# CSU-KangHu/HiTE

Measured on AMD Instinct MI355X. Metric: candidate TE boundaries/sec on 1 Gbp synthetic genome (fine stage: copy finding+gather+align+vote+judge), higher is better.
Workload: dtype u8; 1 GPU; C3: 1000 Mbp synthetic genome, 2500 TIR + 2500 LTR families, 50000 candidates/GPU judged as TIR (copy finding by minimizer-index lookup inside the timed step; index build 0.0 s untimed); genome_bp=1000000000, candidates_per_gpu=50000, candidate_bases=192511237, copies=799813, copy_table=found, is_te=34225, parallelism=replicated genome, candidates per rank x1, all-gather of 32-B calls

## Files before the change

hite_amd/_lib.py:

```python
import ctypes as C
import os

import numpy as np

_HERE = os.path.dirname(os.path.abspath(__file__))
SO_PATH = os.path.join(_HERE, "libhite_gpu.so")

HITE_TE = {"tir": 0, "helitron": 1, "non_ltr": 2}
INFO = {0: "", 1: "nb", 2: "fl1", 3: "EXC"}
HITE_SUBCLUSTER_CHUNK = 64
LTRDEEP_PARAMS, LTRDEEP_ROWS, LTRDEEP_COLS, LTRDEEP_KMER = 40026, 100, 200, 3872


class HiteError(RuntimeError):
    pass


class HiteCall(C.Structure):
    _fields_ = [("is_te", C.c_int32), ("info", C.c_int32), ("row_num", C.c_int32), ("bstart", C.c_int32),
                ("bend", C.c_int32), ("cons_len", C.c_int32), ("cons_off", C.c_int64)]


CALL_DTYPE = np.dtype([("is_te", "<i4"), ("info", "<i4"), ("row_num", "<i4"), ("bstart", "<i4"), ("bend", "<i4"),
                       ("cons_len", "<i4"), ("cons_off", "<i8")])
# ... 42 lines not shown

    def __init__(self, device=0):
        self.lib = load()
        h = C.c_void_p()
        rc = self.lib.hite_ctx_create(int(device), C.byref(h))
        if rc != 0:
            raise HiteError("hite_ctx_create(device=%d) failed: %d (no usable GPU?)" % (device, rc))
        self.h = h
        self.device = device

    def copy_config(self, aligned_interval):
        self._check(self.lib.hite_copy_config_ctx(self.h, -1 if aligned_interval is None else int(bool(aligned_interval))), "hite_copy_config_ctx")

    def fill_config(self, tiles):
        self._check(self.lib.hite_fill_config_ctx(self.h, -1 if tiles is None else int(bool(tiles))), "hite_fill_config_ctx")

    def fill_tile_limits(self):
        out = (C.c_int32 * 4)()
        self._check(self.lib.hite_fill_tile_limits(out), "hite_fill_tile_limits")
        return tuple(out)

    def release_copy_index(self):
        if getattr(self, "_copy_state", None) is not None and getattr(self, "h", None):
            self.lib.hite_copy_index_release(self._copy_state)
        self._copy_state = None

    def close(self):
        self.release_copy_index()
        for lib in list(getattr(self, "_prot_libs", ())) + list(getattr(self, "_ltr_models", ())):
            lib.release()
# ... 1057 lines not shown
```

hite_amd/csrc/hite_align.h:

```cpp
#pragma once
#include "hite_common.h"

int hite_align_run(hite_ctx *ctx, int32_t n_cand, const uint8_t *d_win, const int64_t *d_win_off, const int32_t *d_win_len,
                   const int32_t *d_row_first, int64_t total_rows, const int64_t *d_ops_base, uint16_t *d_ops,
                   int32_t *d_row_dead, int32_t *d_cand_flag, int32_t *d_info, const char *tag, hipStream_t st);
void hite_align_release(hite_ctx *ctx);
```

hite_amd/csrc/hite_align.hip:

```cpp
#include "hite_common.h"
#include "hite_scan.h"
#include "hite_arena.h"
#include "hite_sort.h"
#include "hite_align.h"

#define AL_GAP 3
#define AL_STEER 24
#define AL_MARGIN 48
#define AL_PADR 1056
#define AL_WIDE_NW 64
#define AL_STRIP 16
#define AL_RECB 4096
#define AL_DEFAULT_CAP 8
#define AL_KBINS 2048
#define AL_LANES_MIN_STRIPS 32

struct AlignArgs {
    const uint8_t *win;
    const int64_t *win_off;
    const int32_t *win_len;
    const int32_t *row_first;
    int n_cand;
    const int32_t *row_cand;
    const uint4 *planes;
// ... 1239 lines not shown
                    i -= ups;
                    if (i > 0) {
                        if ((dgv >> ps) & 1ull) { out.put(i - 1, (uint32_t)(j - 1)); i--; j--; }
                        else j--;
                    }
                }
            }
        }
        __syncthreads();
    }
    if (fail) { if (lane == 0) P.st[g] = 1; }
    else out.run(i - 1, i, 0x8000u);
}

__global__ void align_flag_kernel(int64_t nrows, const int32_t *__restrict__ order, const int32_t *__restrict__ strips, AlignArgs P,
                                  int what, int level, int cap, int32_t *__restrict__ flag, int32_t *__restrict__ cols) {
    const int64_t x = (int64_t)blockIdx.x * blockDim.x + threadIdx.x;
    if (x >= nrows) return;
    const int g = order[x];
    int f = 0;
    if (strips[g] > 0) {
        if (what == 0) {
            const int u4 = P.U4[g];
            if (P.st[g] == 0 && u4 >= 0 && u4 + AL_GAP * AL_MARGIN <= 32 * AL_GAP * cap) {
                int first = 8;
                while (32 * AL_GAP * first < u4 + AL_GAP * AL_MARGIN) first *= 2;
                const bool cert = P.U[g] <= P.kst[g];
                f = level >= first && !cert;
            }
        } else if (what == 1) f = P.st[g] == 1;
        else {
            const int u4 = P.U4[g];
            const bool esc = P.st[g] == 0 && u4 >= 0 && u4 + AL_GAP * AL_MARGIN <= 32 * AL_GAP * cap && !(P.U[g] <= P.kst[g]);
            f = what == 2 ? esc : !esc;
        }
    }
    flag[x] = f;
    if (cols) cols[x] = f ? P.win_len[g] + 1 : 0;
}
__global__ void align_compact_kernel(int64_t nrows, const int32_t *__restrict__ order, const int32_t *__restrict__ flag,
                                     const int64_t *__restrict__ pos, int32_t *__restrict__ out, const int64_t *__restrict__ colpos,
                                     int64_t *__restrict__ full_off, int32_t *__restrict__ st) {
    const int64_t x = (int64_t)blockIdx.x * blockDim.x + threadIdx.x;
    if (x >= nrows) return;
    if (flag[x]) {
        const int g = order[x];
        out[pos[x]] = g;
        if (full_off) { full_off[g] = colpos[x]; st[g] = 0; }
    }
}
__global__ void __launch_bounds__(256) align_blockmax_kernel(int64_t cnt, const int32_t *__restrict__ list, const int32_t *__restrict__ strips,
                                                             int32_t *__restrict__ bk) {
    const int64_t x = (int64_t)blockIdx.x * 256 + threadIdx.x;
    const int k = wave_max_i32(x < cnt ? strips[list[x]] : 0);
    if ((threadIdx.x & 63) == 0 && x < cnt) bk[x >> 6] = k;
}
__global__ void align_assign_kernel(int64_t cnt, const int32_t *__restrict__ list, const int64_t *__restrict__ boff, char *region,
                                    unsigned long long *__restrict__ rec) {
    const int64_t x = (int64_t)blockIdx.x * blockDim.x + threadIdx.x;
    if (x < cnt) rec[list[x]] = (unsigned long long)(uintptr_t)(region + boff[x >> 6] * (int64_t)AL_RECB + (x & 63) * 32);
}
struct LaneCost { float thread_chain, lane_chain, thread_work, lane_work; };
__device__ __forceinline__ double lane_cost_at(int64_t k, int64_t nb, const int32_t *bk, const int64_t *boff, const LaneCost c) {
    const double chain_l = k > 0 ? (double)bk[0] * c.lane_chain : 0.0, chain_t = k < nb ? (double)bk[k] * c.thread_chain : 0.0;
// ... 70 lines not shown
    info[g * 5 + 3] = P.kst[g];
    info[g * 5 + 4] = P.lvl[g];
}

struct AlignState {
    Arena arena;
    int64_t *h_pin = nullptr;
    int64_t *d_scal = nullptr;
    int exact_cap = -1;
    int lanes_min = -1;
    float lanes_scale[4] = {1.f, 1.f, 1.f, 1.f};
    bool sort_attr = false;
    hipStream_t st2 = nullptr;
    hipEvent_t ev = nullptr, ev_fork = nullptr, ev_join = nullptr;
    int64_t stats[8] = {0, 0, 0, 0, 0, 0, 0, 0};
};

static hipError_t align_make_stream(hipStream_t *out) {
    int lo = 0, hi = 0;
    if (hipDeviceGetStreamPriorityRange(&lo, &hi) != hipSuccess) { lo = 0; hi = 0; }
    return hipStreamCreateWithPriority(out, hipStreamNonBlocking, hi);
}

static AlignState *align_state(hite_ctx *ctx) {
    if (!ctx->align_state) {
        AlignState *S = new AlignState();
        if (hipHostMalloc((void **)&S->h_pin, 64 * sizeof(int64_t)) != hipSuccess || hipMalloc((void **)&S->d_scal, 64 * sizeof(int64_t)) != hipSuccess ||
            align_make_stream(&S->st2) != hipSuccess || hipEventCreateWithFlags(&S->ev, hipEventDisableTiming) != hipSuccess ||
            hipEventCreateWithFlags(&S->ev_fork, hipEventDisableTiming) != hipSuccess || hipEventCreateWithFlags(&S->ev_join, hipEventDisableTiming) != hipSuccess) {
            delete S;
// ... 49 lines not shown
    return HITE_OK;
}

#define ACHK(x) do { int rc__ = (x); if (rc__) return rc__; } while (0)

template <typename T>
static int aalloc(hite_ctx *ctx, Arena &A, size_t count, T **out) {
    void *p = nullptr;
    int rc = arena_alloc(ctx, A, count * sizeof(T), &p);
    *out = (T *)p;
    return rc;
}

static int build_list(hite_ctx *ctx, AlignState *S, hipStream_t st, int64_t nrows, const int32_t *order, const int32_t *strips,
                      AlignArgs &P, int what, int level, int cap, int32_t *flag, int32_t *cols, int64_t *pos, int64_t *colpos,
                      int64_t *scan_tmp, int32_t *list, int64_t *full_off, int64_t *count, int64_t *total_cols, int slot = 0) {
    const unsigned nb = (unsigned)((nrows + 255) / 256);
    hipLaunchKernelGGL(align_flag_kernel, dim3(nb), dim3(256), 0, st, nrows, order, strips, P, what, level, cap, flag, cols);
    ACHK(scan_excl_buf<int32_t>(ctx, scan_tmp, flag, nrows, pos, st));
    if (cols) ACHK(scan_excl_buf<int32_t>(ctx, scan_tmp, cols, nrows, colpos, st));
    hipLaunchKernelGGL(align_compact_kernel, dim3(nb), dim3(256), 0, st, nrows, order, flag, pos, list, cols ? colpos : nullptr,
                       cols ? full_off : nullptr, P.st);
    HITE_CHECK(ctx, hipMemcpyAsync(S->d_scal + slot, pos + nrows, 8, hipMemcpyDeviceToDevice, st));
    if (cols) HITE_CHECK(ctx, hipMemcpyAsync(S->d_scal + slot + 1, colpos + nrows, 8, hipMemcpyDeviceToDevice, st));
    HITE_CHECK(ctx, hipMemcpyAsync(S->h_pin + slot, S->d_scal + slot, 16, hipMemcpyDeviceToHost, st));
    HITE_CHECK(ctx, hipStreamSynchronize(st));
    *count = S->h_pin[slot];
    if (total_cols) *total_cols = cols ? S->h_pin[slot + 1] : 0;
    return HITE_OK;
}

static int assign_records(hite_ctx *ctx, AlignState *S, hipStream_t st, const int32_t *list, int64_t cnt, const int32_t *strips, int32_t *bk,
                          int64_t *boff, int64_t *scan_tmp, unsigned long long *rec, int slot, int words = 4, int64_t *n_long = nullptr, int64_t *n_long_tb = nullptr) {
    if (n_long) *n_long = 0;
    if (n_long_tb) *n_long_tb = 0;
    if (cnt <= 0) return HITE_OK;
    const int64_t nb = (cnt + 63) / 64;
    hipLaunchKernelGGL(align_blockmax_kernel, dim3((unsigned)((cnt + 255) / 256)), dim3(256), 0, st, cnt, list, strips, bk);
    ACHK(scan_excl_buf<int32_t>(ctx, scan_tmp, bk, nb, boff, st));
    HITE_CHECK(ctx, hipMemcpyAsync(S->d_scal + slot, boff + nb, 8, hipMemcpyDeviceToDevice, st));
    const bool lanes = n_long && S->lanes_min != -2;
    if (lanes) {
        LaneCost fwd4 = {5440.f, 3200.f, 4.3f, 12.5f}, fwd8 = {7040.f, 3200.f, 13.75f, 25.f}, tb = {6880.f, 530.f, 4.3f, 21.5f};
// ... 4 lines not shown
    }
    HITE_CHECK(ctx, hipMemcpyAsync(S->h_pin + slot, S->d_scal + slot, 24, hipMemcpyDeviceToHost, st));
    HITE_CHECK(ctx, hipStreamSynchronize(st));
    const int64_t block_strips = S->h_pin[slot];
    if (lanes) {
        const int64_t v = S->h_pin[slot + 1] * 64, vt = S->h_pin[slot + 2] * 64;
        *n_long = v < cnt ? v : cnt;
        if (n_long_tb) *n_long_tb = vt < cnt ? vt : cnt;
    }
    char *region;
    ACHK(aalloc(ctx, S->arena, (size_t)block_strips * AL_RECB + 256, &region));
    hipLaunchKernelGGL(align_assign_kernel, dim3((unsigned)((cnt + 255) / 256)), dim3(256), 0, st, cnt, list, boff, region, rec);
    return HITE_OK;
}

int hite_align_run(hite_ctx *ctx, int32_t n_cand, const uint8_t *d_win, const int64_t *d_win_off, const int32_t *d_win_len,
                   const int32_t *d_row_first, int64_t total_rows, const int64_t *d_ops_base, uint16_t *d_ops,
                   int32_t *d_row_dead, int32_t *d_cand_flag, int32_t *d_info, const char *tag, hipStream_t st) {
    if (!ctx || n_cand < 0 || total_rows < 0 || total_rows > 0x7fffffff) return HITE_EINVAL;
    if (n_cand == 0 || total_rows == 0) return HITE_OK;
    AlignState *S = align_state(ctx);
    if (!S) return HITE_ENOMEM;
    Arena &A = S->arena;
    ACHK(arena_reset(ctx, A, true));
    const int cap = S->exact_cap;
    AlignArgs P;
    memset(&P, 0, sizeof P);
    P.win = d_win; P.win_off = d_win_off; P.win_len = d_win_len; P.row_first = d_row_first; P.n_cand = n_cand;
    P.ops_base = d_ops_base; P.ops = d_ops;
    int32_t *row_cand, *strips, *order, *pwords, *flag, *flag2, *cols, *list, *list_esc, *list_fin;
    unsigned long long *skeys;
    int64_t *plane_off, *pos, *pos2, *colpos, *scan_tmp, *scan_tmp2, *full_off, *boff, *boff2;
    int32_t *bk, *bk2;
    unsigned long long *rec;
// ... 140 lines not shown
            snprintf(lname, sizeof lname, "align_tb_strips%s", tag ? tag : "");
            const int tl = hite_prof_begin(ctx, lname, s2);
            hipLaunchKernelGGL(align_tb_strips_kernel, dim3((unsigned)nltb), dim3(64), 0, s2, P, order, (int)nltb);
            hite_prof_end(ctx, tl, s2);
            HITE_CHECK(ctx, hipEventRecord(S->ev_join, s2));
        }
        if (nrows > nltb) {
            tk = hite_prof_begin(ctx, name, st);
            hipLaunchKernelGGL(align_tb_kernel, dim3((unsigned)((nrows - nltb + 63) / 64)), dim3(64), 0, st, P, order + nltb, (int)(nrows - nltb));
            hite_prof_end(ctx, tk, st);
        }
        if (nltb > 0) HITE_CHECK(ctx, hipStreamWaitEvent(st, S->ev_join, 0));
    }
    HITE_CHECK(ctx, hipGetLastError());
    {
        int64_t cnt = 0, tcols = 0;
        ACHK(build_list(ctx, S, st, total_rows, order, strips, P, 1, 0, cap, flag, cols, pos, colpos, scan_tmp, list, full_off, &cnt, &tcols));
        if (cnt > 0) {
            tk = hite_prof_begin(ctx, "align_fallback", st);
            ACHK(aalloc(ctx, A, (size_t)tcols * 2 * AL_WIDE_NW + 64, &P.fullbuf));
            ACHK(aalloc(ctx, A, (size_t)tcols + 16, &P.fullt));
            hipLaunchKernelGGL(align_wide_fwd_kernel, dim3((unsigned)cnt), dim3(64), 0, st, P, list, (int)cnt);
            hipLaunchKernelGGL(align_wide_tb_kernel, dim3((unsigned)cnt), dim3(64), 0, st, P, list, (int)cnt);
            hite_prof_end(ctx, tk, st);
        }
    }
    HITE_CHECK(ctx, hipMemsetAsync(S->d_scal, 0, 64, st));
    hipLaunchKernelGGL(align_stats_kernel, dim3((unsigned)(total_rows + 255 < 1024 * 256 ? (total_rows + 255) / 256 : 1024)), dim3(256), 0, st, total_rows, strips, P, d_row_dead, d_cand_flag,
                       (unsigned long long *)S->d_scal);
    if (d_info) hipLaunchKernelGGL(align_info_kernel, dim3((unsigned)((total_rows + 255) / 256)), dim3(256), 0, st, total_rows, P, d_info);
    HITE_CHECK(ctx, hipMemcpyAsync(S->h_pin, S->d_scal, 56, hipMemcpyDeviceToHost, st));
    HITE_CHECK(ctx, hipStreamSynchronize(st));
    for (int q = 0; q < 7; q++) S->stats[q] += S->h_pin[q];
    HITE_CHECK(ctx, hipGetLastError());
    return HITE_OK;
}
```

hite_amd/csrc/hite_common.h:

```cpp
#pragma once
#include <hip/hip_runtime.h>
#include <stdint.h>
#include <stdio.h>
#include <string.h>
#include <stdlib.h>
#include "../../include/hite_gpu.h"

#define HITE_WAVE 64
#define HITE_BLOCK 256

#define JUDGE_CLS_BLOCK 0
#define JUDGE_CLS_WAVE 1
#define JUDGE_CLS_LDS 2
#define JUDGE_LDS_WAVE_SIZES 3
#define JUDGE_LDS_BLOCK_SIZES 2
#define JUDGE_NCLS (JUDGE_CLS_LDS + JUDGE_LDS_WAVE_SIZES + JUDGE_LDS_BLOCK_SIZES)
#define HITE_AUX_STREAMS (JUDGE_NCLS - 1)
struct JudgeFuse {
    const uint8_t *win;
    const int64_t *win_off;
    const int32_t *win_len;
    const int32_t *row_first;
    const int64_t *ops_base;
    const uint16_t *ops;
// ... 22 lines not shown
    int prof_on;
    int prof_n;
    char prof_name[64][32];
    double prof_ms[64];
    int64_t prof_count[64];
    int prof_pending;
    void *prof_ev[512][2];
    int prof_stage[512];
    void *align_state;
    const int32_t *d_msa_row_map;
    const int32_t *d_msa_rows_eff;
    uint32_t *d_msa_lay;
    int msa_long;
    int msa_max_len;
    int32_t fill_tiles;
    const int64_t *d_msa_win_off;
    const int32_t *d_msa_win_len;
    const uint32_t *d_msa_pads;
    int32_t copy_interval;
    int32_t *d_contig_rank;
    void *aux_stream[HITE_AUX_STREAMS];
    void *aux_fork;
    void *aux_join[HITE_AUX_STREAMS];
    int32_t seed_rank, seed_world;
    const uint8_t *d_judge_cls;
    JudgeFuse judge_fuse;
    void *fmea_arena;
    int32_t subcluster_chunk;
    int64_t subcluster_batch_bytes;
    int64_t framecluster_batch_bytes;
    int64_t pairhsp_batch_pairs;
    int64_t ltrscan_batch_bytes;
    int64_t annot_batch_bytes;
    int64_t ltrdeep_batch;
};
void hite_fmea_release(hite_ctx *ctx);
int hite_aux_streams(hite_ctx *ctx, int k, hipStream_t *st, hipEvent_t *fork_ev, hipEvent_t *join_ev);

int hite_prof_begin(hite_ctx *ctx, const char *name, hipStream_t st);
void hite_prof_end(hite_ctx *ctx, int token, hipStream_t st);
void hite_prof_resolve(hite_ctx *ctx);

#define HITE_CHECK(ctx, call)                                                                         \
    do {                                                                                              \
        hipError_t e__ = (call);                                                                      \
        if (e__ != hipSuccess) {                                                                      \
            if (ctx) snprintf((ctx)->err, sizeof((ctx)->err), "%s:%d %s: %s", __FILE__, __LINE__, #call, \
                              hipGetErrorString(e__));                                                \
            return HITE_EHIP;                                                                         \
        }                                                                                             \
    } while (0)
// ... 98 lines not shown
```

hite_amd/csrc/hite_ctx.hip:

```cpp
#include "hite_common.h"
#include "hite_hostbuf.h"
#include "hite_align.h"
#include "hite_genome.h"

extern "C" int hite_version(void) { return 1; }

extern "C" int hite_ctx_create(int device_id, hite_ctx **out) {
    if (!out) return HITE_EINVAL;
    int ndev = 0;
    if (hipGetDeviceCount(&ndev) != hipSuccess || ndev <= 0) return HITE_ENODEV;
    if (device_id < 0 || device_id >= ndev) return HITE_EINVAL;
    hite_ctx *c = (hite_ctx *)calloc(1, sizeof(hite_ctx));
    if (!c) return HITE_ENOMEM;
    c->device = device_id;
    c->copy_interval = -1;
    c->fill_tiles = -1;
    c->subcluster_chunk = HITE_SUBCLUSTER_CHUNK;
    if (const char *e = getenv("HITE_SUBCLUSTER_CHUNK_ROWS")) {
        const long v = strtol(e, nullptr, 10);
        if (v >= 1 && v <= HITE_SUBCLUSTER_CHUNK) c->subcluster_chunk = (int32_t)v;
    }
    if (const char *e = getenv("HITE_SUBCLUSTER_BATCH_BYTES")) {
        const long long v = strtoll(e, nullptr, 10);
        if (v >= 1) c->subcluster_batch_bytes = (int64_t)v;
    }
    if (const char *e = getenv("HITE_FRAMECLUSTER_BATCH_BYTES")) {
        const long long v = strtoll(e, nullptr, 10);
        if (v >= 1 && v <= ((long long)1 << 30)) c->framecluster_batch_bytes = (int64_t)v;
    }
    if (const char *e = getenv("HITE_PAIRHSP_BATCH_PAIRS")) {
        const long long v = strtoll(e, nullptr, 10);
// ... 38 lines not shown
    free(c->mask_log);
    hite_align_release(c);
    hite_fmea_release(c);
    if (c->d_scratch) (void)hipFree(c->d_scratch);
    if (c->d_scratch2) (void)hipFree(c->d_scratch2);
    if (c->d_contig_rank) (void)hipFree(c->d_contig_rank);
    if (c->aux_fork) (void)hipEventDestroy((hipEvent_t)c->aux_fork);
    for (int i = 0; i < HITE_AUX_STREAMS; i++) {
        if (c->aux_join[i]) (void)hipEventDestroy((hipEvent_t)c->aux_join[i]);
        if (c->aux_stream[i]) (void)hipStreamDestroy((hipStream_t)c->aux_stream[i]);
    }
    free(c);
}

extern "C" const char *hite_last_error(hite_ctx *c) { return c ? c->err : "null ctx"; }

extern "C" int hite_set_contig_order(hite_ctx *ctx, const int32_t *rank, int32_t n) {
    if (!ctx) return HITE_EINVAL;
    HITE_CHECK(ctx, hipSetDevice(ctx->device));
    if (ctx->d_contig_rank) { (void)hipFree(ctx->d_contig_rank); ctx->d_contig_rank = nullptr; }
    if (!rank || n <= 0 || n != ctx->n_contigs) return rank && n > 0 ? HITE_EINVAL : HITE_OK;
    HITE_CHECK(ctx, hipMalloc((void **)&ctx->d_contig_rank, (size_t)n * 4));
    HITE_CHECK(ctx, hipMemcpy(ctx->d_contig_rank, rank, (size_t)n * 4, hipMemcpyHostToDevice));
    return HITE_OK;
}

int hite_aux_streams(hite_ctx *ctx, int k, hipStream_t *st, hipEvent_t *fork_ev, hipEvent_t *join_ev) {
    if (k < 0 || k > HITE_AUX_STREAMS) return HITE_EINVAL;
    if (!ctx->aux_fork) {
        hipStream_t s[HITE_AUX_STREAMS] = {};
// ... 399 lines not shown
```

hite_amd/csrc/hite_msa.hip:

```cpp
#include "hite_common.h"
#include "hite_hostbuf.h"
#include "hite_align.h"
#include "hite_scan.h"
#include "hite_fill.h"
#include "hite_fill_tile.h"

#define MSA_MAXR 128

struct MsaParams {
    int n;
    int64_t total_rows;
    const uint8_t *win;
    const int64_t *win_off;
    const int32_t *win_len;
    const int32_t *row_first;
    const int64_t *ops_base;
    uint16_t *ops;
    int32_t *cols_out;
    int32_t *status;
    const int32_t *row_map;
    const int32_t *rows_eff;
    const uint32_t *pads;
    uint32_t *lay;
};

__device__ __forceinline__ int msa_rows(const int32_t *__restrict__ rows_eff, const int32_t *__restrict__ row_first, int c) {
    return rows_eff ? rows_eff[c] : row_first[c + 1] - row_first[c];
}
__device__ __forceinline__ int msa_src(const int32_t *__restrict__ row_map, int64_t g0, int r) {
    return row_map ? row_map[g0 + r] - (int)g0 : r;
}

__device__ __forceinline__ int row_ins_s(const uint16_t *__restrict__ rop, int p, int m, int nrow, int start) {
    int prev_end = start;
    if (p > 0) { unsigned o = rop[p - 1]; prev_end = (int)(o & 0x7fff) + ((o >> 15) ? 0 : 1); }
    int q = p < m ? (int)(rop[p] & 0x7fff) : nrow;
    return q - prev_end;
}
__device__ __forceinline__ int row_ins(const uint16_t *__restrict__ rop, int p, int m, int nrow) {
    const unsigned o = rop[p - 1];
    const int prev_end = (int)(o & 0x7fff) + ((o >> 15) ? 0 : 1);
    int q = p < m ? (int)(rop[p] & 0x7fff) : nrow;
    return q - prev_end;
}

__global__ void __launch_bounds__(256) star_layout_kernel(MsaParams P) {
    __shared__ int s_scan[8];
    const int c = blockIdx.x;
    if (c >= P.n) return;
    const int64_t g0 = P.row_first[c];
    const int R = msa_rows(P.rows_eff, P.row_first, c);
    if (R <= 0) { if (threadIdx.x == 0) P.cols_out[c] = 0; return; }
    const int m = P.win_len[g0];
    uint16_t *ops = P.ops + P.ops_base[c];
    uint16_t *insmax = ops;
    uint16_t *bstart = ops + (int64_t)R * (m + 1);
    if (P.status[c]) { if (threadIdx.x == 0) P.cols_out[c] = 0; return; }
    int running = 0;
    for (int base = 0; base <= m; base += 256) {
        int p = base + threadIdx.x;
        int mx = 0;
        if (p <= m) for (int r = 1; r < R; r++) {
            const int sr = msa_src(P.row_map, g0, r);
            int v = row_ins_s(ops + (int64_t)r * (m + 1), p, m, P.win_len[g0 + sr], P.pads ? (int)(P.pads[g0 + sr] & 0xffffu) : 0);
// ... 60 lines not shown
            const int bs = bstart[p], im = insmax[p];
            const int rp = q - ins;
            for (int k = 0; k < im; k++) row[bs + k] = k < ins ? b[rp + k] : (uint8_t)'-';
            if (p < m) row[bs + im] = gap ? (uint8_t)'-' : b[q];
        }
    }
}

#define LAY_KW_LIST 256
#ifndef LAY_ROWS
#define LAY_ROWS 4
#endif
__device__ __forceinline__ unsigned long long lay_ld8(const uint16_t *p) { unsigned long long v; __builtin_memcpy(&v, p, 8); return v; }

__global__ void __launch_bounds__(256) star_layout_sparse_kernel(MsaParams P, int32_t *__restrict__ new_cols,
                                                                 int32_t *__restrict__ last_extra) {
    __shared__ int s_scan[8];
    __shared__ int s_mxm;
    const int c = blockIdx.x;
    if (c >= P.n) return;
    const int64_t g0 = P.row_first[c];
    const int R = msa_rows(P.rows_eff, P.row_first, c);
    if (R <= 0 || P.status[c]) { if (threadIdx.x == 0) { P.cols_out[c] = 0; new_cols[c] = 0; last_extra[c] = -1; } return; }
    const int m = P.win_len[g0];
    uint16_t *ops = P.ops + P.ops_base[c];
    uint32_t *lay = P.lay + (P.ops_base[c] >> 1);
    const int h = (R + 1) >> 1;
    __shared__ int s_wl[MSA_MAXR];
    __shared__ int s_nkw;
    __shared__ unsigned short s_kwlist[LAY_KW_LIST], s_kwres[4 * 256];
    for (int r = threadIdx.x; r < R && r < MSA_MAXR; r += 256) s_wl[r] = P.win_len[g0 + msa_src(P.row_map, g0, r)];
    if (threadIdx.x == 0) s_mxm = 0;
    __syncthreads();
    const int64_t rs = m + 1;
    {
// ... 294 lines not shown
        if (!step_row(S2, S0, S1, V1, V0)) break;
    }
    while (bad) {
        const int k = __builtin_ctzll(bad), rr = rbase + k * step;
        bad &= bad - 1;
        const RowWin rw = row_win(k);
        ft_cells_direct(out + (int64_t)rr * C, rw.b, rw.n, ops + rr * rs, lay, m, le, rr == 0, P0, pl + 1, lane);
    }
  }
}

__global__ void __launch_bounds__(256) msa_compact_rows_kernel(int n, const int32_t *__restrict__ row_first,
                                                               const int32_t *__restrict__ win_len, const int64_t *__restrict__ ops_base,
                                                               uint16_t *__restrict__ ops_all, const int32_t *__restrict__ cand_flag,
                                                               const int32_t *__restrict__ row_dead, int32_t *__restrict__ row_map,
                                                               int32_t *__restrict__ rows_eff) {
    const int c = blockIdx.x;
    if (c >= n) return;
    const int g0 = row_first[c], R = row_first[c + 1] - g0;
    if (R <= 0) { if (threadIdx.x == 0) rows_eff[c] = 0; return; }
    if (cand_flag[c] != 2) {
        for (int r = threadIdx.x; r < R; r += 256) row_map[g0 + r] = g0 + r;
        if (threadIdx.x == 0) rows_eff[c] = R;
        return;
    }
    const int m = win_len[g0];
    uint16_t *ops = ops_all + ops_base[c];
    int k = 0;
    for (int r = 0; r < R; r++) {
        if (row_dead[g0 + r]) continue;
        if (k != r) for (int p = threadIdx.x; p <= m; p += 256) ops[(int64_t)k * (m + 1) + p] = ops[(int64_t)r * (m + 1) + p];
        if (threadIdx.x == 0) row_map[g0 + k] = g0 + r;
        k++;
// ... 10 lines not shown
__global__ void row_pad_scan_kernel(int64_t total_rows, const uint8_t *__restrict__ win, const int64_t *__restrict__ win_off,
                                    const int32_t *__restrict__ win_len, int32_t *__restrict__ len2, uint32_t *__restrict__ pads) {
    const int64_t g = (int64_t)blockIdx.x * blockDim.x + threadIdx.x;
    if (g >= total_rows) return;
    const uint8_t *b = win + win_off[g];
    const int n = win_len[g];
    int pf = 0, pb = 0;
    if (n > 0 && HITE_IS_ROW_PAD(b[0])) { pf = 1; while (pf < n && HITE_IS_ROW_PAD(b[pf])) pf++; }
    if (pf < n && HITE_IS_ROW_PAD(b[n - 1])) { pb = 1; while (pf + pb < n && HITE_IS_ROW_PAD(b[n - 1 - pb])) pb++; }
    len2[g] = n - pb;
    pads[g] = (uint32_t)pf | ((uint32_t)pb << 16);
}
__global__ void __launch_bounds__(256) ops_pad_fix_kernel(int n, const int32_t *__restrict__ row_first, const int32_t *__restrict__ win_len,
                                                          const int64_t *__restrict__ ops_base, uint16_t *__restrict__ ops_all,
                                                          const uint32_t *__restrict__ pads, const int32_t *__restrict__ row_map,
                                                          const int32_t *__restrict__ rows_eff, int32_t *__restrict__ len2) {
    const int c = blockIdx.x;
    if (c >= n) return;
    const int g0 = row_first[c];
    const int R = rows_eff ? rows_eff[c] : row_first[c + 1] - g0;
    if (R >= 1 && threadIdx.x == 0) len2[g0] = win_len[g0];
    if (R <= 1) return;
    const int m = win_len[g0];
    uint16_t *ops = ops_all + ops_base[c];
    const int lane = threadIdx.x & 63;
    for (int k = 1 + (int)(threadIdx.x >> 6); k < R; k += 4) {
        const int src = row_map ? row_map[g0 + k] : g0 + k;
        const uint32_t pd = pads[src];
        const int pf = (int)(pd & 0xffffu), pb = (int)(pd >> 16), hi = win_len[src] - pb;
        uint16_t *o = ops + (int64_t)k * (m + 1);
        if (lane == 0) o[-1] = (uint16_t)(0x8000u | (unsigned)pf);
        if (pf) {
            for (int base = 0; base < m; base += 64) {
// ... 23 lines not shown
    const size_t ops_bytes = ((size_t)ops_elems * 2 + 255) & ~(size_t)255;
    const size_t rows_bytes = ((size_t)total_rows * 4 + 255) & ~(size_t)255, cand_bytes = ((size_t)n * 4 + 255) & ~(size_t)255;
    void *opsb = nullptr;
    const size_t lay_bytes = d_new_cols ? (((size_t)ops_elems / 2 + 32768 + 16) * 4 + 255) & ~(size_t)255 : 0;
    int rc = hite_scratch2_reserve(ctx, ops_bytes + 2 * rows_bytes + 2 * cand_bytes + lay_bytes + 2 * rows_bytes + 256, &opsb);
    if (rc) return rc;
    uint8_t *base = (uint8_t *)opsb;
    int32_t *row_dead = (int32_t *)(base + ops_bytes), *row_map = (int32_t *)(base + ops_bytes + rows_bytes);
    int32_t *rows_eff = (int32_t *)(base + ops_bytes + 2 * rows_bytes), *cand_flag = (int32_t *)(base + ops_bytes + 2 * rows_bytes + cand_bytes);
    hipStream_t st = (hipStream_t)stream;
    HITE_CHECK(ctx, hipMemsetAsync(d_status, 0, (size_t)n * 4, st));
    HITE_CHECK(ctx, hipMemsetAsync(cand_flag, 0, (size_t)n * 4, st));
    int64_t before[8], after[8];
    rc = hite_align_stats(ctx, before, 0);
    if (rc) return rc;
    rc = hite_align_run(ctx, n, d_win, d_win_off, d_win_len, d_row_first, total_rows, d_ops_base, (uint16_t *)opsb, row_dead, cand_flag, d_info,
                        max_win_len > 1000 ? "_long" : "_short", st);
    if (rc) return rc;
    rc = hite_align_stats(ctx, after, 0);
    if (rc) return rc;
    const bool dropped = after[4] > before[4];
    int32_t *len2 = (int32_t *)(base + ops_bytes + 2 * rows_bytes + 2 * cand_bytes + lay_bytes);
    uint32_t *pads = (uint32_t *)((uint8_t *)len2 + rows_bytes);
    if (total_rows > 0)
        hipLaunchKernelGGL(row_pad_scan_kernel, dim3((unsigned)((total_rows + 255) / 256)), dim3(256), 0, st, total_rows, d_win, d_win_off, d_win_len,
                           len2, pads);
    ctx->d_msa_win_off = d_win_off; ctx->d_msa_win_len = len2; ctx->d_msa_pads = pads; ctx->msa_long = max_win_len > 1536; ctx->msa_max_len = max_win_len;
    MsaParams P;
    P.n = n; P.total_rows = total_rows; P.win = d_win; P.win_off = d_win_off; P.win_len = len2; P.row_first = d_row_first;
    P.ops_base = d_ops_base; P.ops = (uint16_t *)opsb; P.cols_out = d_cols_out; P.status = d_status;
    P.row_map = nullptr; P.rows_eff = nullptr; P.pads = pads;
    P.lay = d_new_cols ? (uint32_t *)(base + ops_bytes + 2 * rows_bytes + 2 * cand_bytes) : nullptr;
    ctx->d_msa_lay = P.lay;
    if (dropped) {
        hipLaunchKernelGGL(msa_compact_rows_kernel, dim3(n), dim3(256), 0, st, n, d_row_first, d_win_len, d_ops_base, (uint16_t *)opsb, cand_flag,
                           row_dead, row_map, rows_eff);
        P.row_map = row_map; P.rows_eff = rows_eff;
    }
    ctx->d_msa_row_map = P.row_map; ctx->d_msa_rows_eff = P.rows_eff;
    hipLaunchKernelGGL(ops_pad_fix_kernel, dim3(n), dim3(256), 0, st, n, d_row_first, d_win_len, d_ops_base, (uint16_t *)opsb, pads, P.row_map,
                       P.rows_eff, len2);
    if (d_rows_out) hipLaunchKernelGGL(msa_rows_out_kernel, dim3((n + 255) / 256), dim3(256), 0, st, n, d_row_first, P.rows_eff, d_rows_out);
    int tk;
    if (d_new_cols) {
        tk = hite_prof_begin(ctx, max_win_len > 1000 ? "star_layout_sparse_kernel_long" : "star_layout_sparse_kernel_short", st);
        hipLaunchKernelGGL(star_layout_sparse_kernel, dim3(n), dim3(256), 0, st, P, d_new_cols, d_last_extra);
    } else {
        tk = hite_prof_begin(ctx, "star_layout_kernel", st);
        hipLaunchKernelGGL(star_layout_kernel, dim3(n), dim3(256), 0, st, P);
    }
    hite_prof_end(ctx, tk, st);
    HITE_CHECK(ctx, hipGetLastError());
    return HITE_OK;
}

extern "C" int hite_star_msa_dev(hite_ctx *ctx, int32_t n, const uint8_t *d_win, const int64_t *d_win_off,
                                 const int32_t *d_win_len, const int32_t *d_row_first, int64_t total_rows, const int64_t *d_ops_base,
                                 int64_t ops_elems, int32_t max_win_len, int32_t *d_cols_out, int32_t *d_status,
                                 int32_t *d_rows_out, void *stream) {
    return star_msa_launch(ctx, n, d_win, d_win_off, d_win_len, d_row_first, total_rows, d_ops_base, ops_elems, max_win_len,
                           d_cols_out, d_status, nullptr, nullptr, d_rows_out, nullptr, stream);
}

extern "C" int hite_star_msa_sparse_dev(hite_ctx *ctx, int32_t n, const uint8_t *d_win, const int64_t *d_win_off,
                                        const int32_t *d_win_len, const int32_t *d_row_first, int64_t total_rows,
                                        const int64_t *d_ops_base, int64_t ops_elems, int32_t max_win_len, int32_t *d_cols_out,
// ... 181 lines not shown
```

include/hite_gpu.h:

```cpp
#ifndef HITE_GPU_H
#define HITE_GPU_H
#include <stdint.h>

#ifdef __cplusplus
extern "C" {
#endif

#define HITE_ROW_PAD 0x2e
#define HITE_IS_ROW_PAD(c) (((c) & 0x20u) != 0)

#define HITE_OK 0
#define HITE_EINVAL (-1)
#define HITE_ENOMEM (-2)
#define HITE_EHIP (-3)
#define HITE_ECAP (-4)
#define HITE_ENODEV (-5)

#define HITE_TE_TIR 0
#define HITE_TE_HELITRON 1
#define HITE_TE_NON_LTR 2

#define HITE_INFO_NONE 0
#define HITE_INFO_NB 1
#define HITE_INFO_FL1 2
// ... 289 lines not shown
int hite_star_msa_dev(hite_ctx *ctx, int32_t n, const uint8_t *d_win, const int64_t *d_win_off,
                      const int32_t *d_win_len, const int32_t *d_row_first, int64_t total_rows, const int64_t *d_ops_base, int64_t ops_elems,
                      int32_t max_win_len, int32_t *d_cols_out, int32_t *d_status, int32_t *d_rows_out, void *stream);
int hite_star_msa_fill_dev(hite_ctx *ctx, int32_t n, const uint8_t *d_win, const int64_t *d_win_off,
                           const int32_t *d_win_len, const int32_t *d_row_first, const int64_t *d_ops_base, const int32_t *d_cols,
                           const int64_t *d_msa_off, uint8_t *d_msa, void *stream);
int hite_star_msa_sparse_dev(hite_ctx *ctx, int32_t n, const uint8_t *d_win, const int64_t *d_win_off,
                             const int32_t *d_win_len, const int32_t *d_row_first, int64_t total_rows,
                             const int64_t *d_ops_base, int64_t ops_elems, int32_t max_win_len, int32_t *d_cols_out,
                             int32_t *d_status, int32_t *d_new_cols, int32_t *d_last_extra, int32_t *d_rows_out, void *stream);
int hite_star_msa_fill_sparse_dev(hite_ctx *ctx, int32_t n, const uint8_t *d_win, const int64_t *d_win_off,
                                  const int32_t *d_win_len, const int32_t *d_row_first, const int64_t *d_ops_base,
                                  const int32_t *d_new_cols, const int32_t *d_last_extra, const int64_t *d_msa_off,
                                  uint8_t *d_msa, void *stream);
int hite_fill_config_ctx(hite_ctx *ctx, int32_t mode);
int hite_fill_tile_limits(int32_t out[4]);

int hite_flank_region_align(hite_ctx *ctx, int32_t te_type, int32_t plant, int32_t n_cand, const uint8_t *cand,
                            const int64_t *cand_off, const int32_t *copy_first, int64_t n_copies, const int32_t *contig,
                            const int64_t *start1, const int64_t *end1, const uint8_t *minus, int32_t flank,
                            hite_call *calls, uint8_t *cons, int64_t cons_cap, int64_t *stats_out);
int hite_flank_region_align_dev(hite_ctx *ctx, void **state_io, int32_t te_type, int32_t plant, int32_t n_cand,
                                const uint8_t *d_cand, const int64_t *d_cand_off, const int32_t *d_copy_first,
                                int64_t n_copies, const int32_t *d_contig, const int64_t *d_start1, const int64_t *d_end1,
                                const uint8_t *d_minus, int32_t flank, hite_call *d_calls, uint8_t *d_cons,
                                int64_t cons_cap, int64_t *stats_out, void *stream);
int hite_clip_probe(hite_ctx *ctx, int32_t n_cand, const uint8_t *cand, const int64_t *cand_off, const int32_t *copy_first,
                    int64_t n_copies, const int32_t *contig, const int64_t *start1, const int64_t *end1, const uint8_t *minus,
                    uint32_t *clip_out);
int hite_fine_rows(hite_ctx *ctx, int32_t n_cand, const uint8_t *cand, const int64_t *cand_off, const int32_t *copy_first,
// ... 33 lines not shown
```

Before: 701,200 candidates/s.

## Overlap wide-band alignment fallback with MSA layout of unaffected candidates

Splits the alignment step into begin and finish phases. The wide-band fallback alignment for failed rows now runs on a secondary stream while the MSA compaction, pad fix and star layout proceed on the main stream for candidates with no pending fallback rows. The pending candidates are then processed in a second pass over a compact list after joining. This hides the fallback latency behind the layout work, at the cost of extra kernels, an atomic dead-row count and more bookkeeping. It is enabled by default via an env or ctx toggle.

```diff
diff --git a/hite_amd/_lib.py b/hite_amd/_lib.py
--- a/hite_amd/_lib.py
+++ b/hite_amd/_lib.py
@@ -80,6 +80,9 @@
 
     def fill_config(self, tiles):
         self._check(self.lib.hite_fill_config_ctx(self.h, -1 if tiles is None else int(bool(tiles))), "hite_fill_config_ctx")
+
+    def fallback_overlap(self, mode):
+        self._check(self.lib.hite_fallback_overlap_ctx(self.h, -1 if mode is None or int(mode) < 0 else int(bool(mode))), "hite_fallback_overlap_ctx")
 
     def fill_tile_limits(self):
         out = (C.c_int32 * 4)()
diff --git a/hite_amd/csrc/hite_align.h b/hite_amd/csrc/hite_align.h
--- a/hite_amd/csrc/hite_align.h
+++ b/hite_amd/csrc/hite_align.h
@@ -4,4 +4,12 @@
 int hite_align_run(hite_ctx *ctx, int32_t n_cand, const uint8_t *d_win, const int64_t *d_win_off, const int32_t *d_win_len,
                    const int32_t *d_row_first, int64_t total_rows, const int64_t *d_ops_base, uint16_t *d_ops,
                    int32_t *d_row_dead, int32_t *d_cand_flag, int32_t *d_info, const char *tag, hipStream_t st);
+struct HiteAlignFork {
+    int64_t cnt, dead_before;
+    const int32_t *d_pending, *d_pend_list, *d_pend_count;
+};
+int hite_align_begin(hite_ctx *ctx, int32_t n_cand, const uint8_t *d_win, const int64_t *d_win_off, const int32_t *d_win_len,
+                     const int32_t *d_row_first, int64_t total_rows, const int64_t *d_ops_base, uint16_t *d_ops,
+                     int32_t *d_row_dead, int32_t *d_cand_flag, int32_t *d_info, const char *tag, hipStream_t st, HiteAlignFork *fork);
+int hite_align_finish(hite_ctx *ctx);
 void hite_align_release(hite_ctx *ctx);
diff --git a/hite_amd/csrc/hite_align.hip b/hite_amd/csrc/hite_align.hip
--- a/hite_amd/csrc/hite_align.hip
+++ b/hite_amd/csrc/hite_align.hip
@@ -1277,11 +1277,16 @@
 }
 
 __global__ void align_flag_kernel(int64_t nrows, const int32_t *__restrict__ order, const int32_t *__restrict__ strips, AlignArgs P,
-                                  int what, int level, int cap, int32_t *__restrict__ flag, int32_t *__restrict__ cols) {
+                                  int what, int level, int cap, int32_t *__restrict__ flag, int32_t *__restrict__ cols,
+                                  unsigned long long *__restrict__ dead = nullptr) {
     const int64_t x = (int64_t)blockIdx.x * blockDim.x + threadIdx.x;
     if (x >= nrows) return;
     const int g = order[x];
     int f = 0;
+    if (dead) {
+        const int st = P.st[g];
+        if (strips[g] > 0 ? (st != 0 && st != 1) : g != P.row_first[P.row_cand[g]]) atomicAdd(dead, 1ull);
+    }
     if (strips[g] > 0) {
         if (what == 0) {
             const int u4 = P.U4[g];
@@ -1311,6 +1316,23 @@
         out[pos[x]] = g;
         if (full_off) { full_off[g] = colpos[x]; st[g] = 0; }
     }
+}
+__global__ void align_pending_kernel(int cnt, const int32_t *__restrict__ list, const int32_t *__restrict__ row_cand,
+                                     int32_t *__restrict__ pending, int32_t *__restrict__ pend_list, int32_t *__restrict__ pend_count) {
+    const int x = blockIdx.x * blockDim.x + threadIdx.x;
+    if (x >= cnt) return;
+    const int c = row_cand[list[x]];
+    if (atomicExch(&pending[c], 1) == 0) pend_list[atomicAdd(pend_count, 1)] = c;
+}
+__global__ void align_dead_mark_kernel(int64_t total_rows, const int32_t *__restrict__ strips, AlignArgs P, const int32_t *__restrict__ pending,
+                                       int32_t *__restrict__ row_dead, int32_t *__restrict__ cand_status) {
+    const int64_t g = (int64_t)blockIdx.x * blockDim.x + threadIdx.x;
+    if (g >= total_rows) return;
+    const int c = P.row_cand[g];
+    if (pending[c]) return;
+    const bool dead = strips[g] > 0 ? P.st[g] != 0 : g != P.row_first[c];
+    row_dead[g] = dead;
+    if (dead) atomicExch(&cand_status[c], 2);
 }
 __global__ void __launch_bounds__(256) align_blockmax_kernel(int64_t cnt, const int32_t *__restrict__ list, const int32_t *__restrict__ strips,
                                                              int32_t *__restrict__ bk) {
@@ -1411,6 +1433,12 @@
     hipStream_t st2 = nullptr;
     hipEvent_t ev = nullptr, ev_fork = nullptr, ev_join = nullptr;
     int64_t stats[8] = {0, 0, 0, 0, 0, 0, 0, 0};
+    bool open = false, forked = false;
+    AlignArgs P;
+    int64_t total_rows = 0;
+    const int32_t *strips = nullptr;
+    int32_t *row_dead = nullptr, *cand_flag = nullptr, *info = nullptr;
+    hipStream_t st = nullptr;
 };
 
 static hipError_t align_make_stream(hipStream_t *out) {
@@ -1490,19 +1518,23 @@
 
 static int build_list(hite_ctx *ctx, AlignState *S, hipStream_t st, int64_t nrows, const int32_t *order, const int32_t *strips,
                       AlignArgs &P, int what, int level, int cap, int32_t *flag, int32_t *cols, int64_t *pos, int64_t *colpos,
-                      int64_t *scan_tmp, int32_t *list, int64_t *full_off, int64_t *count, int64_t *total_cols, int slot = 0) {
+                      int64_t *scan_tmp, int32_t *list, int64_t *full_off, int64_t *count, int64_t *total_cols, int slot = 0,
+                      int64_t *dead = nullptr) {
     const unsigned nb = (unsigned)((nrows + 255) / 256);
-    hipLaunchKernelGGL(align_flag_kernel, dim3(nb), dim3(256), 0, st, nrows, order, strips, P, what, level, cap, flag, cols);
+    if (dead) HITE_CHECK(ctx, hipMemsetAsync(S->d_scal + slot + 2, 0, 8, st));
+    hipLaunchKernelGGL(align_flag_kernel, dim3(nb), dim3(256), 0, st, nrows, order, strips, P, what, level, cap, flag, cols,
+                       dead ? (unsigned long long *)(S->d_scal + slot + 2) : nullptr);
     ACHK(scan_excl_buf<int32_t>(ctx, scan_tmp, flag, nrows, pos, st));
     if (cols) ACHK(scan_excl_buf<int32_t>(ctx, scan_tmp, cols, nrows, colpos, st));
     hipLaunchKernelGGL(align_compact_kernel, dim3(nb), dim3(256), 0, st, nrows, order, flag, pos, list, cols ? colpos : nullptr,
                        cols ? full_off : nullptr, P.st);
     HITE_CHECK(ctx, hipMemcpyAsync(S->d_scal + slot, pos + nrows, 8, hipMemcpyDeviceToDevice, st));
     if (cols) HITE_CHECK(ctx, hipMemcpyAsync(S->d_scal + slot + 1, colpos + nrows, 8, hipMemcpyDeviceToDevice, st));
-    HITE_CHECK(ctx, hipMemcpyAsync(S->h_pin + slot, S->d_scal + slot, 16, hipMemcpyDeviceToHost, st));
+    HITE_CHECK(ctx, hipMemcpyAsync(S->h_pin + slot, S->d_scal + slot, dead ? 24 : 16, hipMemcpyDeviceToHost, st));
     HITE_CHECK(ctx, hipStreamSynchronize(st));
     *count = S->h_pin[slot];
     if (total_cols) *total_cols = cols ? S->h_pin[slot + 1] : 0;
+    if (dead) *dead = S->h_pin[slot + 2];
     return HITE_OK;
 }
 
@@ -1537,10 +1569,13 @@
     return HITE_OK;
 }
 
-int hite_align_run(hite_ctx *ctx, int32_t n_cand, const uint8_t *d_win, const int64_t *d_win_off, const int32_t *d_win_len,
-                   const int32_t *d_row_first, int64_t total_rows, const int64_t *d_ops_base, uint16_t *d_ops,
-                   int32_t *d_row_dead, int32_t *d_cand_flag, int32_t *d_info, const char *tag, hipStream_t st) {
+int hite_align_begin(hite_ctx *ctx, int32_t n_cand, const uint8_t *d_win, const int64_t *d_win_off, const int32_t *d_win_len,
+                     const int32_t *d_row_first, int64_t total_rows, const int64_t *d_ops_base, uint16_t *d_ops,
+                     int32_t *d_row_dead, int32_t *d_cand_flag, int32_t *d_info, const char *tag, hipStream_t st, HiteAlignFork *fork) {
+    if (fork) memset(fork, 0, sizeof *fork);
     if (!ctx || n_cand < 0 || total_rows < 0 || total_rows > 0x7fffffff) return HITE_EINVAL;
+    if (fork && (!d_row_dead || !d_cand_flag)) return HITE_EINVAL;
+    if (ctx->align_state) { ((AlignState *)ctx->align_state)->open = false; ((AlignState *)ctx->align_state)->forked = false; }
     if (n_cand == 0 || total_rows == 0) return HITE_OK;
     AlignState *S = align_state(ctx);
     if (!S) return HITE_ENOMEM;
@@ -1711,17 +1746,58 @@
     }
     HITE_CHECK(ctx, hipGetLastError());
     {
-        int64_t cnt = 0, tcols = 0;
-        ACHK(build_list(ctx, S, st, total_rows, order, strips, P, 1, 0, cap, flag, cols, pos, colpos, scan_tmp, list, full_off, &cnt, &tcols));
-        if (cnt > 0) {
+        int64_t cnt = 0, tcols = 0, dead = 0;
+        ACHK(build_list(ctx, S, st, total_rows, order, strips, P, 1, 0, cap, flag, cols, pos, colpos, scan_tmp, list, full_off, &cnt, &tcols, 0,
+                        fork ? &dead : nullptr));
+        if (cnt > 0 && !fork) {
             tk = hite_prof_begin(ctx, "align_fallback", st);
             ACHK(aalloc(ctx, A, (size_t)tcols * 2 * AL_WIDE_NW + 64, &P.fullbuf));
             ACHK(aalloc(ctx, A, (size_t)tcols + 16, &P.fullt));
             hipLaunchKernelGGL(align_wide_fwd_kernel, dim3((unsigned)cnt), dim3(64), 0, st, P, list, (int)cnt);
             hipLaunchKernelGGL(align_wide_tb_kernel, dim3((unsigned)cnt), dim3(64), 0, st, P, list, (int)cnt);
             hite_prof_end(ctx, tk, st);
-        }
-    }
+        } else if (cnt > 0) {
+            int32_t *pending, *pend_list, *pend_count;
+            ACHK(aalloc(ctx, A, (size_t)tcols * 2 * AL_WIDE_NW + 64, &P.fullbuf));
+            ACHK(aalloc(ctx, A, (size_t)tcols + 16, &P.fullt));
+            ACHK(aalloc(ctx, A, (size_t)n_cand, &pending));
+            ACHK(aalloc(ctx, A, (size_t)cnt, &pend_list));
+            ACHK(aalloc(ctx, A, (size_t)1, &pend_count));
+            HITE_CHECK(ctx, hipEventRecord(S->ev_fork, st));
+            HITE_CHECK(ctx, hipStreamWaitEvent(s2, S->ev_fork, 0));
+            const int tl = hite_prof_begin(ctx, "align_fallback", s2);
+            hipLaunchKernelGGL(align_wide_fwd_kernel, dim3((unsigned)cnt), dim3(64), 0, s2, P, list, (int)cnt);
+            hipLaunchKernelGGL(align_wide_tb_kernel, dim3((unsigned)cnt), dim3(64), 0, s2, P, list, (int)cnt);
+            hite_prof_end(ctx, tl, s2);
+            HITE_CHECK(ctx, hipEventRecord(S->ev_join, s2));
+            HITE_CHECK(ctx, hipMemsetAsync(pending, 0, (size_t)n_cand * 4, st));
+            HITE_CHECK(ctx, hipMemsetAsync(pend_count, 0, 4, st));
+            hipLaunchKernelGGL(align_pending_kernel, dim3((unsigned)((cnt + 255) / 256)), dim3(256), 0, st, (int)cnt, list, row_cand, pending, pend_list, pend_count);
+            if (dead > 0)
+                hipLaunchKernelGGL(align_dead_mark_kernel, dim3((unsigned)((total_rows + 255) / 256)), dim3(256), 0, st, total_rows, strips, P, pending,
+                                   d_row_dead, d_cand_flag);
+            S->forked = true;
+            fork->cnt = cnt; fork->dead_before = dead; fork->d_pending = pending; fork->d_pend_list = pend_list; fork->d_pend_count = pend_count;
+        }
+    }
+    HITE_CHECK(ctx, hipGetLastError());
+    S->P = P; S->total_rows = total_rows; S->strips = strips; S->row_dead = d_row_dead; S->cand_flag = d_cand_flag; S->info = d_info; S->st = st;
+    S->open = true;
+    return HITE_OK;
+}
+
+int hite_align_finish(hite_ctx *ctx) {
+    if (!ctx) return HITE_EINVAL;
+    AlignState *S = (AlignState *)ctx->align_state;
+    if (!S || !S->open) return HITE_OK;
+    S->open = false;
+    const AlignArgs &P = S->P;
+    const int64_t total_rows = S->total_rows;
+    const int32_t *strips = S->strips;
+    int32_t *d_row_dead = S->row_dead, *d_cand_flag = S->cand_flag, *d_info = S->info;
+    hipStream_t st = S->st;
+    if (S->forked) HITE_CHECK(ctx, hipStreamWaitEvent(st, S->ev_join, 0));
+    S->forked = false;
     HITE_CHECK(ctx, hipMemsetAsync(S->d_scal, 0, 64, st));
     hipLaunchKernelGGL(align_stats_kernel, dim3((unsigned)(total_rows + 255 < 1024 * 256 ? (total_rows + 255) / 256 : 1024)), dim3(256), 0, st, total_rows, strips, P, d_row_dead, d_cand_flag,
                        (unsigned long long *)S->d_scal);
@@ -1732,3 +1808,11 @@
     HITE_CHECK(ctx, hipGetLastError());
     return HITE_OK;
 }
+
+int hite_align_run(hite_ctx *ctx, int32_t n_cand, const uint8_t *d_win, const int64_t *d_win_off, const int32_t *d_win_len,
+                   const int32_t *d_row_first, int64_t total_rows, const int64_t *d_ops_base, uint16_t *d_ops,
+                   int32_t *d_row_dead, int32_t *d_cand_flag, int32_t *d_info, const char *tag, hipStream_t st) {
+    ACHK(hite_align_begin(ctx, n_cand, d_win, d_win_off, d_win_len, d_row_first, total_rows, d_ops_base, d_ops, d_row_dead, d_cand_flag, d_info,
+                          tag, st, nullptr));
+    return hite_align_finish(ctx);
+}
diff --git a/hite_amd/csrc/hite_common.h b/hite_amd/csrc/hite_common.h
--- a/hite_amd/csrc/hite_common.h
+++ b/hite_amd/csrc/hite_common.h
@@ -60,6 +60,7 @@
     int msa_long;
     int msa_max_len;
     int32_t fill_tiles;
+    int32_t fallback_overlap;
     const int64_t *d_msa_win_off;
     const int32_t *d_msa_win_len;
     const uint32_t *d_msa_pads;
@@ -81,6 +82,7 @@
     int64_t ltrdeep_batch;
 };
 void hite_fmea_release(hite_ctx *ctx);
+int hite_fallback_overlap_mode(const hite_ctx *ctx);
 int hite_aux_streams(hite_ctx *ctx, int k, hipStream_t *st, hipEvent_t *fork_ev, hipEvent_t *join_ev);
 
 int hite_prof_begin(hite_ctx *ctx, const char *name, hipStream_t st);
diff --git a/hite_amd/csrc/hite_ctx.hip b/hite_amd/csrc/hite_ctx.hip
--- a/hite_amd/csrc/hite_ctx.hip
+++ b/hite_amd/csrc/hite_ctx.hip
@@ -15,6 +15,7 @@
     c->device = device_id;
     c->copy_interval = -1;
     c->fill_tiles = -1;
+    c->fallback_overlap = -1;
     c->subcluster_chunk = HITE_SUBCLUSTER_CHUNK;
     if (const char *e = getenv("HITE_SUBCLUSTER_CHUNK_ROWS")) {
         const long v = strtol(e, nullptr, 10);
@@ -83,6 +84,23 @@
 }
 
 extern "C" const char *hite_last_error(hite_ctx *c) { return c ? c->err : "null ctx"; }
+
+static int g_fallback_overlap = -1;
+int hite_fallback_overlap_mode(const hite_ctx *ctx) {
+    if (ctx->fallback_overlap >= 0) return ctx->fallback_overlap;
+    int v = __atomic_load_n(&g_fallback_overlap, __ATOMIC_RELAXED);
+    if (v < 0) {
+        const char *e = getenv("HITE_FALLBACK_OVERLAP");
+        v = (e && !strcmp(e, "0")) ? 0 : 1;
+        __atomic_store_n(&g_fallback_overlap, v, __ATOMIC_RELAXED);
+    }
+    return v;
+}
+extern "C" int hite_fallback_overlap_ctx(hite_ctx *ctx, int32_t mode) {
+    if (!ctx || mode < -1 || mode > 1) return HITE_EINVAL;
+    ctx->fallback_overlap = mode;
+    return HITE_OK;
+}
 
 extern "C" int hite_set_contig_order(hite_ctx *ctx, const int32_t *rank, int32_t n) {
     if (!ctx) return HITE_EINVAL;
diff --git a/hite_amd/csrc/hite_msa.hip b/hite_amd/csrc/hite_msa.hip
--- a/hite_amd/csrc/hite_msa.hip
+++ b/hite_amd/csrc/hite_msa.hip
@@ -31,6 +31,14 @@
     return row_map ? row_map[g0 + r] - (int)g0 : r;
 }
 
+__device__ __forceinline__ int msa_block_cand(int n, const int32_t *__restrict__ pending, const int32_t *__restrict__ pend_list,
+                                              const int32_t *__restrict__ pend_count) {
+    const int b = blockIdx.x;
+    if (pend_list) return b < *pend_count ? pend_list[b] : -1;
+    if (b >= n || (pending && pending[b])) return -1;
+    return b;
+}
+
 __device__ __forceinline__ int row_ins_s(const uint16_t *__restrict__ rop, int p, int m, int nrow, int start) {
     int prev_end = start;
     if (p > 0) { unsigned o = rop[p - 1]; prev_end = (int)(o & 0x7fff) + ((o >> 15) ? 0 : 1); }
@@ -44,10 +52,11 @@
     return q - prev_end;
 }
 
-__global__ void __launch_bounds__(256) star_layout_kernel(MsaParams P) {
+__global__ void __launch_bounds__(256) star_layout_kernel(MsaParams P, const int32_t *__restrict__ pending, const int32_t *__restrict__ pend_list,
+                                                          const int32_t *__restrict__ pend_count) {
     __shared__ int s_scan[8];
-    const int c = blockIdx.x;
-    if (c >= P.n) return;
+    const int c = msa_block_cand(P.n, pending, pend_list, pend_count);
+    if (c < 0) return;
     const int64_t g0 = P.row_first[c];
     const int R = msa_rows(P.rows_eff, P.row_first, c);
     if (R <= 0) { if (threadIdx.x == 0) P.cols_out[c] = 0; return; }
@@ -138,11 +147,12 @@
 __device__ __forceinline__ unsigned long long lay_ld8(const uint16_t *p) { unsigned long long v; __builtin_memcpy(&v, p, 8); return v; }
 
 __global__ void __launch_bounds__(256) star_layout_sparse_kernel(MsaParams P, int32_t *__restrict__ new_cols,
-                                                                 int32_t *__restrict__ last_extra) {
+                                                                 int32_t *__restrict__ last_extra, const int32_t *__restrict__ pending,
+                                                                 const int32_t *__restrict__ pend_list, const int32_t *__restrict__ pend_count) {
     __shared__ int s_scan[8];
     __shared__ int s_mxm;
-    const int c = blockIdx.x;
-    if (c >= P.n) return;
+    const int c = msa_block_cand(P.n, pending, pend_list, pend_count);
+    if (c < 0) return;
     const int64_t g0 = P.row_first[c];
     const int R = msa_rows(P.rows_eff, P.row_first, c);
     if (R <= 0 || P.status[c]) { if (threadIdx.x == 0) { P.cols_out[c] = 0; new_cols[c] = 0; last_extra[c] = -1; } return; }
@@ -467,9 +477,10 @@
                                                                const int32_t *__restrict__ win_len, const int64_t *__restrict__ ops_base,
                                                                uint16_t *__restrict__ ops_all, const int32_t *__restrict__ cand_flag,
                                                                const int32_t *__restrict__ row_dead, int32_t *__restrict__ row_map,
-                                                               int32_t *__restrict__ rows_eff) {
-    const int c = blockIdx.x;
-    if (c >= n) return;
+                                                               int32_t *__restrict__ rows_eff, const int32_t *__restrict__ pending,
+                                                               const int32_t *__restrict__ pend_list, const int32_t *__restrict__ pend_count) {
+    const int c = msa_block_cand(n, pending, pend_list, pend_count);
+    if (c < 0) return;
     const int g0 = row_first[c], R = row_first[c + 1] - g0;
     if (R <= 0) { if (threadIdx.x == 0) rows_eff[c] = 0; return; }
     if (cand_flag[c] != 2) {
@@ -510,9 +521,11 @@
 __global__ void __launch_bounds__(256) ops_pad_fix_kernel(int n, const int32_t *__restrict__ row_first, const int32_t *__restrict__ win_len,
                                                           const int64_t *__restrict__ ops_base, uint16_t *__restrict__ ops_all,
                                                           const uint32_t *__restrict__ pads, const int32_t *__restrict__ row_map,
-                                                          const int32_t *__restrict__ rows_eff, int32_t *__restrict__ len2) {
-    const int c = blockIdx.x;
-    if (c >= n) return;
+                                                          const int32_t *__restrict__ rows_eff, int32_t *__restrict__ len2,
+                                                          const int32_t *__restrict__ pending, const int32_t *__restrict__ pend_list,
+                                                          const int32_t *__restrict__ pend_count) {
+    const int c = msa_block_cand(n, pending, pend_list, pend_count);
+    if (c < 0) return;
     const int g0 = row_first[c];
     const int R = rows_eff ? rows_eff[c] : row_first[c + 1] - g0;
     if (R >= 1 && threadIdx.x == 0) len2[g0] = win_len[g0];
@@ -566,12 +579,19 @@
     int64_t before[8], after[8];
     rc = hite_align_stats(ctx, before, 0);
     if (rc) return rc;
-    rc = hite_align_run(ctx, n, d_win, d_win_off, d_win_len, d_row_first, total_rows, d_ops_base, (uint16_t *)opsb, row_dead, cand_flag, d_info,
-                        max_win_len > 1000 ? "_long" : "_short", st);
+    HiteAlignFork F;
+    memset(&F, 0, sizeof F);
+    rc = hite_align_begin(ctx, n, d_win, d_win_off, d_win_len, d_row_first, total_rows, d_ops_base, (uint16_t *)opsb, row_dead, cand_flag, d_info,
+                          max_win_len > 1000 ? "_long" : "_short", st, hite_fallback_overlap_mode(ctx) ? &F : nullptr);
     if (rc) return rc;
-    rc = hite_align_stats(ctx, after, 0);
-    if (rc) return rc;
-    const bool dropped = after[4] > before[4];
+    const bool forked = F.cnt > 0;
+    if (!forked) {
+        rc = hite_align_finish(ctx);
+        if (rc) return rc;
+        rc = hite_align_stats(ctx, after, 0);
+        if (rc) return rc;
+    }
+    bool dropped = forked ? F.dead_before > 0 : after[4] > before[4];
     int32_t *len2 = (int32_t *)(base + ops_bytes + 2 * rows_bytes + 2 * cand_bytes + lay_bytes);
     uint32_t *pads = (uint32_t *)((uint8_t *)len2 + rows_bytes);
     if (total_rows > 0)
@@ -584,24 +604,42 @@
     P.row_map = nullptr; P.rows_eff = nullptr; P.pads = pads;
     P.lay = d_new_cols ? (uint32_t *)(base + ops_bytes + 2 * rows_bytes + 2 * cand_bytes) : nullptr;
     ctx->d_msa_lay = P.lay;
-    if (dropped) {
-        hipLaunchKernelGGL(msa_compact_rows_kernel, dim3(n), dim3(256), 0, st, n, d_row_first, d_win_len, d_ops_base, (uint16_t *)opsb, cand_flag,
-                           row_dead, row_map, rows_eff);
-        P.row_map = row_map; P.rows_eff = rows_eff;
+    auto pass = [&](bool compact, const int32_t *pending, const int32_t *plist, const int32_t *pcount, unsigned grid, bool rows_out) {
+        if (compact) {
+            hipLaunchKernelGGL(msa_compact_rows_kernel, dim3(grid), dim3(256), 0, st, n, d_row_first, d_win_len, d_ops_base, (uint16_t *)opsb, cand_flag,
+                               row_dead, row_map, rows_eff, pending, plist, pcount);
+            P.row_map = row_map; P.rows_eff = rows_eff;
+        }
+        hipLaunchKernelGGL(ops_pad_fix_kernel, dim3(grid), dim3(256), 0, st, n, d_row_first, d_win_len, d_ops_base, (uint16_t *)opsb, pads, P.row_map,
+                           P.rows_eff, len2, pending, plist, pcount);
+        if (rows_out && d_rows_out) hipLaunchKernelGGL(msa_rows_out_kernel, dim3((n + 255) / 256), dim3(256), 0, st, n, d_row_first, P.rows_eff, d_rows_out);
+        int tk;
+        if (d_new_cols) {
+            tk = hite_prof_begin(ctx, max_win_len > 1000 ? "star_layout_sparse_kernel_long" : "star_layout_sparse_kernel_short", st);
+            hipLaunchKernelGGL(star_layout_sparse_kernel, dim3(grid), dim3(256), 0, st, P, d_new_cols, d_last_extra, pending, plist, pcount);
+        } else {
+            tk = hite_prof_begin(ctx, "star_layout_kernel", st);
+            hipLaunchKernelGGL(star_layout_kernel, dim3(grid), dim3(256), 0, st, P, pending, plist, pcount);
+        }
+        hite_prof_end(ctx, tk, st);
+    };
+    if (!forked) pass(dropped, nullptr, nullptr, nullptr, (unsigned)n, true);
+    else {
+        const bool compact_win = dropped;
+        pass(compact_win, F.d_pending, nullptr, nullptr, (unsigned)n, false);
+        rc = hite_align_finish(ctx);
+        if (rc) return rc;
+        rc = hite_align_stats(ctx, after, 0);
+        if (rc) return rc;
+        dropped = after[4] > before[4];
+        if (dropped && !compact_win) {
+            hipLaunchKernelGGL(msa_compact_rows_kernel, dim3(n), dim3(256), 0, st, n, d_row_first, d_win_len, d_ops_base, (uint16_t *)opsb, cand_flag,
+                               row_dead, row_map, rows_eff, nullptr, nullptr, nullptr);
+            P.row_map = row_map; P.rows_eff = rows_eff;
+        }
+        pass(dropped && compact_win, nullptr, F.d_pend_list, F.d_pend_count, (unsigned)F.cnt, true);
     }
     ctx->d_msa_row_map = P.row_map; ctx->d_msa_rows_eff = P.rows_eff;
-    hipLaunchKernelGGL(ops_pad_fix_kernel, dim3(n), dim3(256), 0, st, n, d_row_first, d_win_len, d_ops_base, (uint16_t *)opsb, pads, P.row_map,
-                       P.rows_eff, len2);
-    if (d_rows_out) hipLaunchKernelGGL(msa_rows_out_kernel, dim3((n + 255) / 256), dim3(256), 0, st, n, d_row_first, P.rows_eff, d_rows_out);
-    int tk;
-    if (d_new_cols) {
-        tk = hite_prof_begin(ctx, max_win_len > 1000 ? "star_layout_sparse_kernel_long" : "star_layout_sparse_kernel_short", st);
-        hipLaunchKernelGGL(star_layout_sparse_kernel, dim3(n), dim3(256), 0, st, P, d_new_cols, d_last_extra);
-    } else {
-        tk = hite_prof_begin(ctx, "star_layout_kernel", st);
-        hipLaunchKernelGGL(star_layout_kernel, dim3(n), dim3(256), 0, st, P);
-    }
-    hite_prof_end(ctx, tk, st);
     HITE_CHECK(ctx, hipGetLastError());
     return HITE_OK;
 }
diff --git a/include/hite_gpu.h b/include/hite_gpu.h
--- a/include/hite_gpu.h
+++ b/include/hite_gpu.h
@@ -327,6 +327,7 @@
                                   const int32_t *d_new_cols, const int32_t *d_last_extra, const int64_t *d_msa_off,
                                   uint8_t *d_msa, void *stream);
 int hite_fill_config_ctx(hite_ctx *ctx, int32_t mode);
+int hite_fallback_overlap_ctx(hite_ctx *ctx, int32_t mode);
 int hite_fill_tile_limits(int32_t out[4]);
 
 int hite_flank_region_align(hite_ctx *ctx, int32_t te_type, int32_t plant, int32_t n_cand, const uint8_t *cand,
```

New measurement: 718,700 candidates/s (median of 6 runs). +2.5%, better.
